# elfi-dev/elfi

Hardware: AMD Instinct MI355X
Metric: ABC distances/sec (higher is better)
Workload: dtype f64

## Files before the change

elfi_amd/csrc/gp_fit.hip:

```cpp
#include "gp.hpp"
#include "mfma_f64.hpp"
#include "sweep_sched.hpp"

#include <map>
#include <memory>
#include <mutex>

namespace elfihip {

struct GramArgs {
  const double* X;
  const double* x2;
  const double* y;
  double* A;
  int64_t lda, n, np;
  int dp;
  double var, neg_half_inv_ls2, bias, diag_add;
  int* info;
  int ninfo;
};

__global__ __launch_bounds__(256) void gram_kernel(GramArgs G) {
  extern __shared__ __align__(16) double sm[];
  const int pitch = G.dp + 1;
// ... 511 lines not shown
    } else {
      idx -= tA + m;
      const int r = idx / m;
      cblk = c0 + (idx - r * m);
      Ap = P.WT + ((int64_t)r * NB) * P.lda + (int64_t)P.ku0 * NB;
      C = P.WT + ((int64_t)r * NB) * P.lda + (int64_t)cblk * NB;
      beta0 = (r >= P.ku0);
    }
  }
  const double* Bp = P.A + ((int64_t)cblk * NB) * P.lda + (int64_t)P.ku0 * NB;
  GemmAcc acc;
  acc.zero();
  if (same)
    gemm_tile_nt<true>(acc, Ap, P.lda, Bp, P.lda, 0, P.kun * NB, lds);
  else
    gemm_tile_nt<false>(acc, Ap, P.lda, Bp, P.lda, 0, P.kun * NB, lds);
  if (beta0)
    acc_foreach(acc, [&](int row, int col, double v) { C[(int64_t)row * P.lda + col] = -v; });
  else
    acc_foreach(acc, [&](int row, int col, double v) { C[(int64_t)row * P.lda + col] -= v; });
}

__global__ __launch_bounds__(256) void trailing_update_col_kernel(PanelArgs P, int cblk) {
  extern __shared__ __align__(16) double lds[];
  cblk += blockIdx.y;
  const int rb = blockIdx.x >> 2, sub = blockIdx.x & 3;
  const int mrows = P.nb - cblk;
  if (rb >= mrows + 1 + P.ku0 + P.kun) return;
  const double* Ap;
  double* C;
  bool beta0 = false;
  if (rb < mrows) {
    const int ib = cblk + rb;
    Ap = P.A + ((int64_t)ib * NB) * P.lda + (int64_t)P.ku0 * NB;
    C = P.A + ((int64_t)ib * NB) * P.lda + (int64_t)cblk * NB;
  } else if (rb == mrows) {
    Ap = P.A + ((int64_t)P.nb * NB) * P.lda + (int64_t)P.ku0 * NB;
    C = P.A + ((int64_t)P.nb * NB) * P.lda + (int64_t)cblk * NB;
  } else {
    const int r = rb - mrows - 1;
    Ap = P.WT + ((int64_t)r * NB) * P.lda + (int64_t)P.ku0 * NB;
    C = P.WT + ((int64_t)r * NB) * P.lda + (int64_t)cblk * NB;
    beta0 = (r >= P.ku0);
  }
  Ap += (int64_t)sub * 32 * P.lda;
  C += (int64_t)sub * 32 * P.lda;
  const double* Bp = P.A + ((int64_t)cblk * NB) * P.lda + (int64_t)P.ku0 * NB;
  GemmAcc32 acc;
  acc.zero();
  gemm_tile32_nt(acc, Ap, P.lda, Bp, P.lda, 0, P.kun * NB, lds);
  if (beta0)
    acc32_foreach(acc, [&](int row, int col, double v) { C[(int64_t)row * P.lda + col] = -v; });
  else
    acc32_foreach(acc, [&](int row, int col, double v) { C[(int64_t)row * P.lda + col] -= v; });
}

template <int KUN, bool WT>
__device__ __forceinline__ void lookahead_tile_body(const PanelArgs& P, int cblk, int lb, double* lds) {
  const int t = threadIdx.x, l = t & 63, w = t >> 6;
  const int rb = lb >> 4, sub = (lb >> 2) & 3, cs = lb & 3;
  const int mrows = P.nb - cblk;
  if (rb >= mrows + 1 + P.ku0 + P.kun) return;
  const double* Ap;
  double* C;
  bool beta0 = false;
  if (rb < mrows) {
    const int ib = cblk + rb;
    Ap = P.A + ((int64_t)ib * NB) * P.lda + (int64_t)P.ku0 * NB;
    C = P.A + ((int64_t)ib * NB) * P.lda + (int64_t)cblk * NB;
  } else if (rb == mrows) {
    Ap = P.A + ((int64_t)P.nb * NB) * P.lda + (int64_t)P.ku0 * NB;
    C = P.A + ((int64_t)P.nb * NB) * P.lda + (int64_t)cblk * NB;
  } else {
    const int r = rb - mrows - 1;
    Ap = P.WT + ((int64_t)r * NB) * P.lda + (int64_t)P.ku0 * NB;
    C = P.WT + ((int64_t)r * NB) * P.lda + (int64_t)cblk * NB;
    beta0 = (r >= P.ku0);
  }
  Ap += (int64_t)sub * 32 * P.lda;
  C += (int64_t)sub * 32 * P.lda + cs * 32;
  const double* Bp = P.A + ((int64_t)cblk * NB + cs * 32) * P.lda + (int64_t)P.ku0 * NB;
  constexpr int KW = 32 * KUN;
  constexpr int NO = 4;
  const int kb = w * KW + 2 * (l >> 4);
  const double* pa = Ap + (int64_t)(l & 15) * P.lda + kb;
  const double* pb = Bp + (int64_t)(l & 15) * P.lda + kb;
  double2 a[2][2][NO], b[2][2][NO];
  auto load_piece = [&](int buf, int piece) {
#pragma unroll
    for (int o = 0; o < NO; ++o)
#pragma unroll
      for (int i = 0; i < 2; ++i) {
        a[buf][i][o] = *reinterpret_cast<const double2*>(pa + (int64_t)i * 16 * P.lda + 32 * piece + 8 * o);
        b[buf][i][o] = *reinterpret_cast<const double2*>(pb + (int64_t)i * 16 * P.lda + 32 * piece + 8 * o);
      }
  };
  load_piece(0, 0);
  if (KUN > 1) load_piece(1, 1);
  double cv[4];
#pragma unroll
  for (int u = 0; u < 4; ++u) {
    const int e = t + 256 * u;
    cv[u] = beta0 ? 0.0 : C[(int64_t)(e >> 5) * P.lda + (e & 31)];
  }
  v4d acc[2][2];
#pragma unroll
  for (int i = 0; i < 2; ++i)
#pragma unroll
    for (int j = 0; j < 2; ++j) acc[i][j] = (v4d){0.0, 0.0, 0.0, 0.0};
#pragma unroll
  for (int piece = 0; piece < KUN; ++piece) {
    const int buf = piece & 1;
#pragma unroll
    for (int o = 0; o < NO; ++o)
#pragma unroll
      for (int i = 0; i < 2; ++i)
#pragma unroll
        for (int j = 0; j < 2; ++j) {
          acc[i][j] = __builtin_amdgcn_mfma_f64_16x16x4f64(a[buf][i][o].x, b[buf][j][o].x, acc[i][j], 0, 0, 0);
          acc[i][j] = __builtin_amdgcn_mfma_f64_16x16x4f64(a[buf][i][o].y, b[buf][j][o].y, acc[i][j], 0, 0, 0);
        }
    if (piece + 2 < KUN) load_piece(buf, piece + 2);
  }
  constexpr int TP = 33;
  double* part = lds + w * 32 * TP;
#pragma unroll
  for (int i = 0; i < 2; ++i)
#pragma unroll
    for (int j = 0; j < 2; ++j)
#pragma unroll
      for (int r = 0; r < 4; ++r) part[(i * 16 + (l >> 4) + 4 * r) * TP + j * 16 + (l & 15)] = acc[i][j][r];
  __syncthreads();
#pragma unroll
  for (int u = 0; u < 4; ++u) {
    const int e = t + 256 * u;
    const int o = (e >> 5) * TP + (e & 31);
    const double s = ((lds[o] + lds[32 * TP + o]) + lds[2 * 32 * TP + o]) + lds[3 * 32 * TP + o];
    if (WT)
      store_wt_f64(C + (int64_t)(e >> 5) * P.lda + (e & 31), cv[u] - s);
    else
      C[(int64_t)(e >> 5) * P.lda + (e & 31)] = cv[u] - s;
  }
}

template <int KUN>
__global__ __launch_bounds__(256) void lookahead_tile_kernel(PanelArgs P, int cblk) {
  extern __shared__ __align__(16) double lds[];
  lookahead_tile_body<KUN, false>(P, cblk + blockIdx.y, (blockIdx.x & 7) * (gridDim.x >> 3) + (blockIdx.x >> 3), lds);
}
constexpr size_t LOOKAHEAD_TILE_LDS = 4 * 32 * 33 * sizeof(double);

constexpr int LOOK_TILES = 36;
constexpr int LOOK_PP = 130;
constexpr size_t PANEL_LOOK_LDS = (2 * 16 * LOOK_PP + 4 * 16 * 17) * sizeof(double);

template <int W>
__device__ __forceinline__ void look_strip_wave(const double* As, int64_t lda, const double* W11, int l, double* Ps,
                                                unsigned* cnt) {
  constexpr int T0 = W, T1 = 7 - W;
  constexpr int O0 = 2 * (T0 + 1), O1 = 2 * (T1 + 1);
  const int q2 = 2 * (l >> 4);
  const double* pa = As + (int64_t)(l & 15) * lda + q2;
  const double* pb0 = W11 + (int64_t)(16 * T0 + (l & 15)) * NB + q2;
  const double* pb1 = W11 + (int64_t)(16 * T1 + (l & 15)) * NB + q2;
  double2 a[O1], b0[O0], b1[O1];
#pragma unroll
  for (int o = 0; o < O1; ++o) a[o] = *reinterpret_cast<const double2*>(pa + 8 * o);
#pragma unroll
  for (int o = 0; o < O0; ++o) b0[o] = *reinterpret_cast<const double2*>(pb0 + 8 * o);
#pragma unroll
  for (int o = 0; o < O1; ++o) b1[o] = *reinterpret_cast<const double2*>(pb1 + 8 * o);
  __builtin_amdgcn_s_waitcnt(WAIT_VMCNT0);
  if (l == 0) __hip_atomic_fetch_add(cnt, 1u, __ATOMIC_RELAXED, __HIP_MEMORY_SCOPE_AGENT);
  v4d c0 = (v4d){0.0, 0.0, 0.0, 0.0}, c1 = c0;
#pragma unroll
  for (int o = 0; o < O1; ++o) {
    if (o < O0) {
      c0 = __builtin_amdgcn_mfma_f64_16x16x4f64(a[o].x, b0[o].x, c0, 0, 0, 0);
      c0 = __builtin_amdgcn_mfma_f64_16x16x4f64(a[o].y, b0[o].y, c0, 0, 0, 0);
    }
    c1 = __builtin_amdgcn_mfma_f64_16x16x4f64(a[o].x, b1[o].x, c1, 0, 0, 0);
    c1 = __builtin_amdgcn_mfma_f64_16x16x4f64(a[o].y, b1[o].y, c1, 0, 0, 0);
  }
  double* po = Ps + (l >> 4) * LOOK_PP + (l & 15);
#pragma unroll
  for (int r = 0; r < 4; ++r) {
    po[4 * r * LOOK_PP + 16 * T0] = c0[r];
    po[4 * r * LOOK_PP + 16 * T1] = c1[r];
  }
}

constexpr unsigned LOOK_ARRIVALS = 28u * 8u + 8u * 4u;

__global__ __launch_bounds__(512) void panel_look_kernel(PanelArgs P, unsigned* cnt, int* info) {
  extern __shared__ __align__(16) double lds[];
  const int t = threadIdx.x, l = t & 63, w = t >> 6, ww = w & 3, half = w >> 2;
  if (blockIdx.x >= LOOK_TILES) {
    const int piece = 2 * (blockIdx.x - LOOK_TILES) + half;
    const int npieces = 8 * P.nb;
    const int pc = piece < npieces ? piece : npieces - 1;
    double* Pb = panel_block(P, pc >> 3) + (int64_t)(pc & 7) * 16 * P.lda;
    unsigned* wait = (pc >> 3) == 0 ? cnt : nullptr;
    switch (ww) {
      case 0: trsm16_wave<0>(Pb, P.lda, P.W11, l, wait, info); break;
      case 1: trsm16_wave<1>(Pb, P.lda, P.W11, l, wait, info); break;
      case 2: trsm16_wave<2>(Pb, P.lda, P.W11, l, wait, info); break;
      default: trsm16_wave<3>(Pb, P.lda, P.W11, l, wait, info); break;
    }
    return;
  }
  int i = 0, b = blockIdx.x;
  while (b > i) {
    b -= i + 1;
    ++i;
  }
  const int j = b;
  const bool diag = i == j;
  const double* Ablk = P.A + ((int64_t)(P.k + 1) * NB) * P.lda + (int64_t)P.k * NB;
  double* C = P.A + ((int64_t)(P.k + 1) * NB + 16 * i) * P.lda + (int64_t)(P.k + 1) * NB + 16 * j;
  double* Pi = lds;
  double* Pj = diag ? lds : lds + 16 * LOOK_PP;
  double* part = lds + 2 * 16 * LOOK_PP;
  double cv = 0.0;
  if (t < 256) cv = C[(int64_t)(t >> 4) * P.lda + (t & 15)];
  if (half == 0 || !diag) {
    const double* As = Ablk + (int64_t)(16 * (half == 0 ? i : j)) * P.lda;
    double* Ps = half == 0 ? Pi : Pj;
    switch (ww) {
      case 0: look_strip_wave<0>(As, P.lda, P.W11, l, Ps, cnt); break;
      case 1: look_strip_wave<1>(As, P.lda, P.W11, l, Ps, cnt); break;
      case 2: look_strip_wave<2>(As, P.lda, P.W11, l, Ps, cnt); break;
      default: look_strip_wave<3>(As, P.lda, P.W11, l, Ps, cnt); break;
    }
  }
  __syncthreads();
  if (half == 0) {
    const int kb = 32 * w + 2 * (l >> 4);
    const double* pa = Pi + (l & 15) * LOOK_PP + kb;
    const double* pb = Pj + (l & 15) * LOOK_PP + kb;
    v4d acc = (v4d){0.0, 0.0, 0.0, 0.0};
#pragma unroll
    for (int o = 0; o < 4; ++o) {
      const double2 a = *reinterpret_cast<const double2*>(pa + 8 * o);
      const double2 bb = *reinterpret_cast<const double2*>(pb + 8 * o);
      acc = __builtin_amdgcn_mfma_f64_16x16x4f64(a.x, bb.x, acc, 0, 0, 0);
      acc = __builtin_amdgcn_mfma_f64_16x16x4f64(a.y, bb.y, acc, 0, 0, 0);
    }
#pragma unroll
    for (int r = 0; r < 4; ++r) part[w * 16 * 17 + ((l >> 4) + 4 * r) * 17 + (l & 15)] = acc[r];
  }
  __syncthreads();
  if (t < 256) {
    const int o = (t >> 4) * 17 + (t & 15);
    const double sum = ((part[o] + part[16 * 17 + o]) + part[2 * 16 * 17 + o]) + part[3 * 16 * 17 + o];
    C[(int64_t)(t >> 4) * P.lda + (t & 15)] = cv - sum;
  }
}

__device__ __noinline__ void potf2_tiles_call(double* Akk, int64_t lda, double* Wkk, int64_t ldw, double* W11, int* info,
                                              int kblock, double* sm) {
  potf2_tiles_body<1024>(Akk, lda, Wkk, ldw, W11, info, kblock, sm);
}
__device__ __noinline__ void potf2_tiles_call_wt(double* Akk, int64_t lda, double* Wkk, int64_t ldw, double* W11, int* info,
                                                 int kblock, double* sm) {
  potf2_tiles_body<1024, true>(Akk, lda, Wkk, ldw, W11, info, kblock, sm);
}

struct StepArgs {
  PanelArgs P;
  double* W11;
  int* info;
  const SweepUnit* units;
  const int32_t* wg_off;
  const SweepUnit* heads;
  unsigned* cnt;
  int nmini;
  int nwg;
};

struct StepUnit {
  const double* Ap;
  const double* Bp;
  double* C;
  double keep;
  int nkt;
  int kt0;
};

__device__ __forceinline__ StepUnit step_decode(const StepArgs& S, const int4 r) {
  const PanelArgs& P = S.P;
  const int row = r.x, c = r.y & 0xffff, kt0 = (r.y >> 16) & 0xffff;
  const int nkt = r.z & 0xffff, half = (r.z >> 16) & 0xff, keep = (r.z >> 24) & 0xff;
  const double* base = row <= P.nb ? P.A + ((int64_t)row * NB) * P.lda : P.WT + ((int64_t)(row - P.nb - 1) * NB) * P.lda;
  StepUnit U;
  U.Ap = base + (int64_t)kt0 * GK2 + (int64_t)half * 64 * P.lda;
  U.C = const_cast<double*>(base) + (int64_t)c * NB + (int64_t)half * 64 * P.lda;
  U.Bp = P.A + ((int64_t)c * NB) * P.lda + (int64_t)kt0 * GK2;
  U.keep = keep ? 1.0 : 0.0;
  U.nkt = nkt;
  U.kt0 = kt0;
  return U;
}

__device__ __forceinline__ StepUnit step_unit(const StepArgs& S, int i) {
  return step_decode(S, *reinterpret_cast<const int4*>(S.units + i));
}

#ifdef ELFIHIP_STEP_STAMP
__device__ long long g_step_stamp[1024 * 8];
__device__ int g_step_stamp_k = 16;
#define SSTAMP(slot) do { if (threadIdx.x == 0 && S.P.k == g_step_stamp_k) g_step_stamp[blockIdx.x * 8 + (slot)] = __builtin_readcyclecounter(); } while (0)
#else
#define SSTAMP(slot) do { } while (0)
#endif

constexpr int STEP_SPIN_LIMIT = 1 << 22;
constexpr int STEP_INFO_TIMEOUT = -1;

__device__ __forceinline__ void step_wait(const unsigned* c, unsigned target, int* info) {
  if (threadIdx.x < 64) {
    if (threadIdx.x == 0) {
      int spins = 0;
      while (__hip_atomic_load(c, __ATOMIC_RELAXED, __HIP_MEMORY_SCOPE_AGENT) < target) {
        if (++spins >= STEP_SPIN_LIMIT) {
          atomicCAS(info, 0, STEP_INFO_TIMEOUT);
          break;
        }
        __builtin_amdgcn_s_sleep(2);
      }
    }
    __builtin_amdgcn_fence(__ATOMIC_ACQUIRE, "agent");
  }
  __syncthreads();
}
__device__ __forceinline__ void step_arrive(unsigned* c, unsigned n, unsigned* c2 = nullptr) {
  asm volatile("s_waitcnt vmcnt(0)" ::: "memory");
  __syncthreads();
  if (threadIdx.x == 0) {
    __hip_atomic_fetch_add(c, n, __ATOMIC_RELAXED, __HIP_MEMORY_SCOPE_AGENT);
    if (c2) __hip_atomic_fetch_add(c2, n, __ATOMIC_RELAXED, __HIP_MEMORY_SCOPE_AGENT);
  }
}

__device__ __forceinline__ void step_solve_piece(const PanelArgs& P, int piece, double* sm) {
  double* Pb = panel_block(P, piece >> 3) + (int64_t)(piece & 7) * 16 * P.lda;
  const int l = threadIdx.x & 63, w = threadIdx.x >> 6;
  const int h = w >> 3, T = w & 7;
  const int O = 2 * (T + 1);
  const int q2 = 2 * (l >> 4);
  const double* pa = Pb + (int64_t)(l & 15) * P.lda + q2 + 64 * h;
  const double* pb = P.W11 + (int64_t)(16 * T + (l & 15)) * NB + q2 + 64 * h;
  double2 a[8], b[8];
#pragma unroll
  for (int j = 0; j < 8; ++j) {
    a[j] = (double2){0.0, 0.0};
    b[j] = (double2){0.0, 0.0};
    if (8 * h + j < O) {
      a[j] = *reinterpret_cast<const double2*>(pa + 8 * j);
      b[j] = *reinterpret_cast<const double2*>(pb + 8 * j);
    }
  }
  v4d c = (v4d){0.0, 0.0, 0.0, 0.0};
#pragma unroll
  for (int j = 0; j < 8; ++j)
    if (8 * h + j < O) {
      c = __builtin_amdgcn_mfma_f64_16x16x4f64(a[j].x, b[j].x, c, 0, 0, 0);
      c = __builtin_amdgcn_mfma_f64_16x16x4f64(a[j].y, b[j].y, c, 0, 0, 0);
    }
  double* part = sm + (T * 64 + l) * 4;
  if (h == 1) {
#pragma unroll
    for (int r = 0; r < 4; ++r) part[r] = c[r];
  }
  __syncthreads();
  if (h == 0) {
    double* po = Pb + (int64_t)(l >> 4) * P.lda + (l & 15) + 16 * T;
#pragma unroll
    for (int r = 0; r < 4; ++r) store_wt_f64(po + (int64_t)(4 * r) * P.lda, c[r] + part[r]);
  }
  __syncthreads();
}

__device__ __forceinline__ void step_tile_pieces(const PanelArgs& P, int pair, double* sm) {
  const int t = threadIdx.x & 255, l = t & 63, w = t >> 6;
  const int g = threadIdx.x >> 8;
  const int lb = 2 * pair + (g & 1);
  const int sub = (lb >> 2) & 3, cs = lb & 3;
  const int cblk = P.k + 1;
  constexpr int TP = 33;
  double* lds = sm + (g & 1) * 4 * 32 * TP;
  const bool on = g < 2;
  const double* Ap = P.A + ((int64_t)cblk * NB + sub * 32) * P.lda + (int64_t)P.k * NB;
  const double* Bp = P.A + ((int64_t)cblk * NB + cs * 32) * P.lda + (int64_t)P.k * NB;
  double* C = P.A + ((int64_t)cblk * NB + sub * 32) * P.lda + (int64_t)cblk * NB + cs * 32;
  double cv[4];
  if (on) {
    const int kb = w * 32 + 2 * (l >> 4);
    const double* pa = Ap + (int64_t)(l & 15) * P.lda + kb;
    const double* pb = Bp + (int64_t)(l & 15) * P.lda + kb;
    double2 a[2][4], b[2][4];
#pragma unroll
    for (int o = 0; o < 4; ++o)
#pragma unroll
      for (int i = 0; i < 2; ++i) {
        a[i][o] = *reinterpret_cast<const double2*>(pa + (int64_t)i * 16 * P.lda + 8 * o);
        b[i][o] = *reinterpret_cast<const double2*>(pb + (int64_t)i * 16 * P.lda + 8 * o);
      }
#pragma unroll
    for (int u = 0; u < 4; ++u) {
      const int e = t + 256 * u;
      cv[u] = C[(int64_t)(e >> 5) * P.lda + (e & 31)];
    }
    v4d acc[2][2];
#pragma unroll
    for (int i = 0; i < 2; ++i)
#pragma unroll
      for (int j = 0; j < 2; ++j) acc[i][j] = (v4d){0.0, 0.0, 0.0, 0.0};
#pragma unroll
    for (int o = 0; o < 4; ++o)
#pragma unroll
      for (int i = 0; i < 2; ++i)
#pragma unroll
        for (int j = 0; j < 2; ++j) {
          acc[i][j] = __builtin_amdgcn_mfma_f64_16x16x4f64(a[i][o].x, b[j][o].x, acc[i][j], 0, 0, 0);
          acc[i][j] = __builtin_amdgcn_mfma_f64_16x16x4f64(a[i][o].y, b[j][o].y, acc[i][j], 0, 0, 0);
        }
    double* part = lds + w * 32 * TP;
#pragma unroll
    for (int i = 0; i < 2; ++i)
#pragma unroll
      for (int j = 0; j < 2; ++j)
#pragma unroll
        for (int r = 0; r < 4; ++r) part[(i * 16 + (l >> 4) + 4 * r) * TP + j * 16 + (l & 15)] = acc[i][j][r];
  }
  __syncthreads();
  if (on) {
#pragma unroll
    for (int u = 0; u < 4; ++u) {
      const int e = t + 256 * u;
      const int o = (e >> 5) * TP + (e & 31);
      const double sres = ((lds[o] + lds[32 * TP + o]) + lds[2 * 32 * TP + o]) + lds[3 * 32 * TP + o];
      store_wt_f64(C + (int64_t)(e >> 5) * P.lda + (e & 31), cv[u] - sres);
    }
  }
}

template <bool CHAINED, bool WT>
__device__ __forceinline__ void step_units(const StepArgs& S, double* sm, int wgi) {
  const PanelArgs& P = S.P;
  constexpr bool chained = CHAINED;
  constexpr int RT = 1;
  constexpr int ROWS = 64 * RT;
  constexpr int BUF = (ROWS + 128) * GLP2;
  const int4 head = *reinterpret_cast<const int4*>(S.heads + wgi);
  int u = S.wg_off[wgi];
  if (head.w <= 0) return;
  const int uend = u + head.w;
  const int t = threadIdx.x, l = t & 63, w = t >> 6;
  const int wr = w >> 2, wc = w & 3;
  const int64_t lda = P.lda;
  const int64_t goff = (int64_t)(t >> 4) * lda + 2 * (t & 15);
  const int doff = (t >> 4) * GLP2 + 2 * (t & 15);
  const int faoff = (wr * 16 * RT + (l & 15)) * GLP2 + 2 * (l >> 4);
  const int fboff = (ROWS + wc * 32 + (l & 15)) * GLP2 + 2 * (l >> 4);
  const int64_t coff = (int64_t)(wr * 16 * RT + (l >> 4)) * lda + wc * 32 + (l & 15);

  StepUnit cur = step_decode(S, head);
  const int kt_new = chained ? 4 * P.k : (1 << 30);
  bool ready = !chained;
  auto need_panel = [&](const StepUnit& U, int kt) {
    if (chained && !ready && U.kt0 + kt >= kt_new) {
      SSTAMP(4);
      step_wait(S.cnt, (unsigned)S.nmini, S.info);
      SSTAMP(5);
      ready = true;
    }
  };
  double2 pa0, pa1, pb0, pb1;
  auto issue = [&](const double* A_, const double* B_) {
    pa0 = *reinterpret_cast<const double2*>(A_ + goff);
    if (RT == 2) pa1 = *reinterpret_cast<const double2*>(A_ + goff + 64 * lda);
    pb0 = *reinterpret_cast<const double2*>(B_ + goff);
    pb1 = *reinterpret_cast<const double2*>(B_ + goff + 64 * lda);
  };
  auto stage = [&](double* buf) {
    double* da = buf + doff;
    *reinterpret_cast<double2*>(da) = pa0;
    if (RT == 2) *reinterpret_cast<double2*>(da + 64 * GLP2) = pa1;
    *reinterpret_cast<double2*>(da + ROWS * GLP2) = pb0;
    *reinterpret_cast<double2*>(da + (ROWS + 64) * GLP2) = pb1;
  };
  pa1 = (double2){0.0, 0.0};
  need_panel(cur, 1);
  issue(cur.Ap, cur.Bp);
  v4d cv[RT][2];
#pragma unroll
  for (int i = 0; i < RT; ++i)
#pragma unroll
    for (int j = 0; j < 2; ++j)
#pragma unroll
      for (int r = 0; r < 4; ++r) cv[i][j][r] = cur.C[coff + (int64_t)(i * 16 + 4 * r) * lda + j * 16];
  int p = 0;
  stage(sm);
  issue(cur.Ap + GK2, cur.Bp + GK2);
  __syncthreads();
  for (;;) {
    const int un = u + 1;
    const bool more = un < uend;
    const StepUnit nxt = more ? step_unit(S, un) : cur;
    v4d acc[RT][2];
#pragma unroll
    for (int i = 0; i < RT; ++i)
#pragma unroll
      for (int j = 0; j < 2; ++j) acc[i][j] = (v4d){0.0, 0.0, 0.0, 0.0};
#pragma unroll 1
    for (int kt = 0; kt < cur.nkt; ++kt) {
      const double* buf = sm + p * BUF;
      if (kt + 1 < cur.nkt || more) {
        stage(sm + (p ^ 1) * BUF);
        const int k2 = kt + 2 - cur.nkt;
        if (k2 < 0) {
          need_panel(cur, kt + 2);
          issue(cur.Ap + (kt + 2) * GK2, cur.Bp + (kt + 2) * GK2);
        } else if (more) {
          need_panel(nxt, k2);
          issue(nxt.Ap + k2 * GK2, nxt.Bp + k2 * GK2);
        }
      }
      const double* fa = buf + faoff;
      const double* fb = buf + fboff;
#pragma unroll
      for (int h = 0; h < 4; ++h) {
        double2 a[RT], bb[2];
#pragma unroll
        for (int i = 0; i < RT; ++i) a[i] = *reinterpret_cast<const double2*>(fa + i * 16 * GLP2 + 8 * h);
#pragma unroll
        for (int j = 0; j < 2; ++j) bb[j] = *reinterpret_cast<const double2*>(fb + j * 16 * GLP2 + 8 * h);
#pragma unroll
        for (int i = 0; i < RT; ++i)
#pragma unroll
          for (int j = 0; j < 2; ++j) {
            acc[i][j] = __builtin_amdgcn_mfma_f64_16x16x4f64(a[i].x, bb[j].x, acc[i][j], 0, 0, 0);
            acc[i][j] = __builtin_amdgcn_mfma_f64_16x16x4f64(a[i].y, bb[j].y, acc[i][j], 0, 0, 0);
          }
      }
      __syncthreads();
      p ^= 1;
    }
    double* cp = cur.C + coff;
#pragma unroll
    for (int i = 0; i < RT; ++i)
#pragma unroll
      for (int j = 0; j < 2; ++j)
#pragma unroll
        for (int r = 0; r < 4; ++r)
          if (WT)
            store_wt_f64(cp + (int64_t)(i * 16 + 4 * r) * lda + j * 16, cur.keep * cv[i][j][r] - acc[i][j][r]);
          else
            cp[(int64_t)(i * 16 + 4 * r) * lda + j * 16] = cur.keep * cv[i][j][r] - acc[i][j][r];
    if (!more) {
      SSTAMP(6);
      break;
    }
    const double* cn = nxt.C + coff;
#pragma unroll
    for (int i = 0; i < RT; ++i)
#pragma unroll
      for (int j = 0; j < 2; ++j)
#pragma unroll
        for (int r = 0; r < 4; ++r) cv[i][j][r] = cn[(int64_t)(i * 16 + 4 * r) * lda + j * 16];
    cur = nxt;
    u = un;
  }
}

template <bool CHAINED>
__device__ __forceinline__ void step_body(const StepArgs& S) {
  extern __shared__ __align__(16) double sm[];
  const PanelArgs& P = S.P;
  constexpr bool chained = CHAINED;
  SSTAMP(0);
  if (blockIdx.x == 0) {
    const int kk = P.k + 1;
    double* Akk = P.A + ((int64_t)kk * NB) * P.lda + (int64_t)kk * NB;
    double* Wkk = P.WT + ((int64_t)kk * NB) * P.lda + (int64_t)kk * NB;
    if (chained) step_wait(S.cnt + 2, 8u, S.info);
    SSTAMP(1);
    if (S.W11) potf2_tiles_call(Akk, P.lda, Wkk, P.lda, S.W11, S.info, kk, sm);
    SSTAMP(2);
    return;
  }
  const int idx = blockIdx.x - 1;
  if (chained) {
    const int lead = S.nwg >= 16 ? 8 : 0;
    if (idx < 8) {
      step_solve_piece(P, idx, sm);
      step_arrive(S.cnt + 1, 1u, S.cnt);
      SSTAMP(1);
    }
    unsigned done = 0;
    if (idx >= lead)
      for (int e = 8 + (idx - lead); e < S.nmini; e += S.nwg - lead) {
        step_solve_piece(P, e, sm);
        ++done;
      }
    if (done) step_arrive(S.cnt, done);
    if (idx >= 8) SSTAMP(1);
    if (idx < 8) {
      step_wait(S.cnt + 1, 8u, S.info);
      SSTAMP(2);
      step_tile_pieces(P, idx, sm);
      step_arrive(S.cnt + 2, 1u);
      SSTAMP(3);
    }
  }
  step_units<CHAINED, false>(S, sm, idx);
}

__global__ __launch_bounds__(1024) void step_kernel(StepArgs S) { step_body<false>(S); }
__global__ __launch_bounds__(1024) void step_chain_kernel(StepArgs S) { step_body<true>(S); }

constexpr size_t STEP_LDS_BYTES = 2 * (64 + 128) * GLP2 * sizeof(double);
static_assert(STEP_LDS_BYTES >= POTF2T_LDS_DOUBLES * sizeof(double) && STEP_LDS_BYTES <= 160 * 1024, "LDS budget");

constexpr int OV_WORDS = 8;
constexpr int OV_POTF2 = 0, OV_PANEL = 1, OV_STRIP = 2, OV_TILE = 3, OV_UPD = 4;
constexpr int OV_AUX_XRANK = 0;
constexpr int OV_AUX_NEXT = 16;
constexpr int OV_AUX_DIAG_XCC = 17;
constexpr int OV_AUX_RESIDENT = 18;
constexpr int OV_AUX_WORDS = 32;
constexpr int OV_TILE_WGS = 16;
constexpr int OV_SPIN_LIMIT = 1 << 20;

__device__ __forceinline__ bool ov_poll(const unsigned* c, unsigned target, int* info, int who = 0) {
  int spins = 0;
  while (__hip_atomic_load(c, __ATOMIC_RELAXED, __HIP_MEMORY_SCOPE_AGENT) < target) {
    ++spins;
    if (spins >= OV_SPIN_LIMIT || ((spins & 31) == 0 && __hip_atomic_load(info + 1, __ATOMIC_RELAXED, __HIP_MEMORY_SCOPE_AGENT) != 0)) {
      if (atomicCAS(info + 1, 0, 1) == 0) {
        info[2] = who;
        info[3] = (int)((__hip_atomic_load(c, __ATOMIC_RELAXED, __HIP_MEMORY_SCOPE_AGENT) << 16) | (target & 0xffffu));
      }
      atomicCAS(info, 0, STEP_INFO_TIMEOUT);
      return false;
    }
    __builtin_amdgcn_s_sleep(8);
  }
  return true;
}
__device__ __forceinline__ bool ov_wait(const unsigned* c0, unsigned t0, const unsigned* c1, unsigned t1, int* info, int* s_ok,
                                        int who) {
  if (threadIdx.x < 64) {
    if (threadIdx.x == 0) {
      bool ok = ov_poll(c0, t0, info, who);
      if (ok && c1) ok = ov_poll(c1, t1, info, who + 1);
      *s_ok = ok ? 1 : 0;
    }
    __builtin_amdgcn_fence(__ATOMIC_ACQUIRE, "agent");
  }
  __syncthreads();
  return *s_ok != 0;
}
__device__ __forceinline__ void ov_arrive(unsigned* c, unsigned* c2 = nullptr) {
  asm volatile("s_waitcnt vmcnt(0)" ::: "memory");
  __syncthreads();
  if (threadIdx.x == 0) {
    __hip_atomic_fetch_add(c, 1u, __ATOMIC_RELAXED, __HIP_MEMORY_SCOPE_AGENT);
    if (c2) __hip_atomic_fetch_add(c2, 1u, __ATOMIC_RELAXED, __HIP_MEMORY_SCOPE_AGENT);
  }
}

struct OvArgs {
  PanelArgs P;
  double* W11;
  int* info;
  unsigned* flags;
  const SweepUnit* units;
  const int32_t* wg_off;
  const SweepUnit* heads;
  unsigned* aux;
  int nwg;
};

__device__ __forceinline__ unsigned ov_xcc_id() { return __builtin_amdgcn_s_getreg((3 << 11) | 20) & 15u; }

__global__ __launch_bounds__(1024) __attribute__((amdgpu_waves_per_eu(5))) void sweep_update_kernel(OvArgs O) {
  extern __shared__ __align__(16) double sm[];
  __shared__ int s_ok;
  __shared__ int s_wgi;
  if (threadIdx.x == 0) {
    __hip_atomic_fetch_add(O.aux + OV_AUX_XRANK + ov_xcc_id(), 1u, __ATOMIC_RELAXED, __HIP_MEMORY_SCOPE_AGENT);
    const int w = (int)__hip_atomic_fetch_add(O.aux + OV_AUX_NEXT, 1u, __ATOMIC_RELAXED, __HIP_MEMORY_SCOPE_AGENT);
    if (w < O.nwg) __hip_atomic_fetch_add(O.aux + OV_AUX_RESIDENT, 1u, __ATOMIC_RELAXED, __HIP_MEMORY_SCOPE_AGENT);
    s_wgi = w;
  }
  __syncthreads();
  const int wgi = s_wgi;
  if (wgi >= O.nwg) return;
  StepArgs S;
  S.P = O.P;
  S.P.kun = 1;
  S.W11 = nullptr;
  S.info = O.info;
  S.units = O.units;
  S.cnt = nullptr;
  S.nmini = 0;
  S.nwg = O.nwg;
  for (int k = 0; k + 1 < O.P.nb; ++k) {
    S.heads = O.heads + (size_t)k * O.nwg;
    const int4 head = *reinterpret_cast<const int4*>(S.heads + wgi);
    if (head.w <= 0) continue;
    unsigned* fl = O.flags + (size_t)OV_WORDS * k;
    if (!ov_wait(fl + OV_PANEL, 8u * (unsigned)O.P.nb, nullptr, 0u, O.info, &s_ok, 1000 + k)) return;
    S.P.k = k;
    S.P.ku0 = k;
    S.wg_off = O.wg_off + (size_t)k * (O.nwg + 1);
    step_units<false, true>(S, sm, wgi);
    ov_arrive(fl + OV_UPD);
  }
}

__global__ __launch_bounds__(1024) void sweep_diag_kernel(OvArgs O) {
  extern __shared__ __align__(16) double sm[];
  __shared__ int s_ok;
  const int wid = __builtin_amdgcn_readfirstlane(threadIdx.x >> 6);
  if (wid >= 11 || wid == 7 || wid == 8) return;
  if (threadIdx.x == 0) {
    __hip_atomic_store(O.aux + OV_AUX_DIAG_XCC, 1u + ov_xcc_id(), __ATOMIC_RELAXED, __HIP_MEMORY_SCOPE_AGENT);
    __hip_atomic_fetch_add(O.aux + OV_AUX_RESIDENT, 1u, __ATOMIC_RELAXED, __HIP_MEMORY_SCOPE_AGENT);
  }
  const PanelArgs& P = O.P;
  for (int k = 0; k + 1 < P.nb; ++k) {
    unsigned* fl = O.flags + (size_t)OV_WORDS * k;
    if (!ov_wait(fl + OV_TILE, (unsigned)OV_TILE_WGS, nullptr, 0u, O.info, &s_ok, 2000 + k)) return;
    const int kk = k + 1;
    double* Akk = P.A + ((int64_t)kk * NB) * P.lda + (int64_t)kk * NB;
    double* Wkk = P.WT + ((int64_t)kk * NB) * P.lda + (int64_t)kk * NB;
    potf2_tiles_call_wt(Akk, P.lda, Wkk, P.lda, O.W11 + (size_t)(kk & 1) * NB * NB, O.info, kk, sm);
    asm volatile("s_waitcnt vmcnt(0)" ::: "memory");
    __syncthreads();
    if (threadIdx.x == 0)
      __hip_atomic_store(fl + OV_WORDS + OV_POTF2, 1u, __ATOMIC_RELAXED, __HIP_MEMORY_SCOPE_AGENT);
  }
}

__global__ __launch_bounds__(256) __attribute__((amdgpu_waves_per_eu(4))) void chain_ov_kernel(PanelArgs P, unsigned* fl, unsigned upd_target, int ntile, int* info) {
  extern __shared__ __align__(16) double lds[];
  __shared__ int s_ok;
  __builtin_amdgcn_s_setprio(3);
  if ((int)blockIdx.x < ntile) {
    if (!ov_wait(fl + OV_STRIP, 8u, nullptr, 0u, info, &s_ok, 5000 + P.k)) return;
    lookahead_tile_body<1, true>(P, P.k + 1, blockIdx.x, lds);
    ov_arrive(fl + OV_TILE);
    return;
  }
  const int b = blockIdx.x - ntile;
  if (P.k > 0 && !ov_wait(fl + OV_POTF2, 1u, fl - OV_WORDS + OV_UPD, upd_target, info, &s_ok, 3000 + 2 * P.k)) return;
  double* Pb = panel_block(P, b >> 3) + (int64_t)(b & 7) * 16 * P.lda;
  const int l = threadIdx.x & 63;
  switch (threadIdx.x >> 6) {
    case 0: trsm16_wave<0, true>(Pb, P.lda, P.W11, l); break;
    case 1: trsm16_wave<1, true>(Pb, P.lda, P.W11, l); break;
    case 2: trsm16_wave<2, true>(Pb, P.lda, P.W11, l); break;
    default: trsm16_wave<3, true>(Pb, P.lda, P.W11, l); break;
  }
  ov_arrive(fl + OV_PANEL, (ntile && b < 8) ? fl + OV_STRIP : nullptr);
}

__global__ __launch_bounds__(64) void ov_gate_kernel(const unsigned* word, unsigned target, int* info, int who) {
  if (threadIdx.x == 0) ov_poll(word, target, info, who);
}

__global__ __launch_bounds__(256) void alpha_logdet_kernel(const double* WT, const double* A, const double* z, double* alpha,
                                                           double* red, const int* info, int64_t n, int64_t np, int64_t lda,
                                                           unsigned long long ticket) {
  if (blockIdx.x == 0) {
    __shared__ double s0[256], s1[256], s2[256], s3[256];
    double a = 0.0, b = 0.0, lo = 1e300, hi = 0.0;
    for (int64_t i = threadIdx.x; i < n; i += 256) {
      const double dg = A[i * lda + i];
      a += log(dg);
      b += z[i] * z[i];
      lo = dg < lo ? dg : lo;
      hi = dg > hi ? dg : hi;
    }
    s0[threadIdx.x] = a;
    s1[threadIdx.x] = b;
    s2[threadIdx.x] = lo;
    s3[threadIdx.x] = hi;
    __syncthreads();
    for (int off = 128; off > 0; off >>= 1) {
      if (threadIdx.x < off) {
        s0[threadIdx.x] += s0[threadIdx.x + off];
        s1[threadIdx.x] += s1[threadIdx.x + off];
        s2[threadIdx.x] = s2[threadIdx.x + off] < s2[threadIdx.x] ? s2[threadIdx.x + off] : s2[threadIdx.x];
        s3[threadIdx.x] = s3[threadIdx.x + off] > s3[threadIdx.x] ? s3[threadIdx.x + off] : s3[threadIdx.x];
      }
      __syncthreads();
    }
    if (threadIdx.x == 0) {
      red[0] = s0[0];
      red[1] = s1[0];
      red[2] = (double)*info;
      red[8] = s2[0];
      red[9] = s3[0];
      post_ticket(red + 15, ticket);
    }
    return;
  }
  const int lane = threadIdx.x & 63;
  const int64_t row = (int64_t)(blockIdx.x - 1) * 4 + (threadIdx.x >> 6);
  double s = 0.0;
  if (row < n) {
    const double* w = WT + row * lda;
    double p[8] = {0.0, 0.0, 0.0, 0.0, 0.0, 0.0, 0.0, 0.0};
    int64_t k = (row & ~(int64_t)63) + lane;
    for (; k + 7 * 64 < n; k += 512) {
      double wv[8], zv[8];
#pragma unroll
      for (int u = 0; u < 8; ++u) {
        wv[u] = w[k + 64 * u];
        zv[u] = z[k + 64 * u];
      }
#pragma unroll
      for (int u = 0; u < 8; ++u) p[u] += (k + 64 * u >= row) ? wv[u] * zv[u] : 0.0;
    }
    double tail = 0.0;
    for (; k < n; k += 64)
      if (k >= row) tail += w[k] * z[k];
    s = (((p[0] + p[1]) + (p[2] + p[3])) + ((p[4] + p[5]) + (p[6] + p[7]))) + tail;
#pragma unroll
    for (int off = 32; off > 0; off >>= 1) s += __shfl_xor(s, off, 64);
  }
  if (lane == 0 && row < np) alpha[row] = s;
}

template <class K>
static int enable_lds(elfihip_ctx* ctx, K k, size_t bytes) {
  ELFIHIP_CHECK_HIP(ctx, hipFuncSetAttribute(reinterpret_cast<const void*>(k),
                                             hipFuncAttributeMaxDynamicSharedMemorySize, (int)bytes));
  return ELFIHIP_OK;
}

static std::mutex g_sched_mutex;
static std::map<std::pair<int, int>, std::shared_ptr<const SweepSchedule>> g_sched_cache;

static std::shared_ptr<const SweepSchedule> sweep_schedule_for(int nb, int nwg, bool far_first) {
  std::lock_guard<std::mutex> lock(g_sched_mutex);
  auto key = std::make_pair(nb, far_first ? -nwg : nwg);
  auto it = g_sched_cache.find(key);
  if (it != g_sched_cache.end()) return it->second;
  auto S = std::make_shared<SweepSchedule>();
  sweep_build(nb, nwg, S.get(), far_first);
  g_sched_cache[key] = S;
  return S;
}

static int sweep_plan(elfihip_gp* gp, int nb, int nwg, bool far_first, hipStream_t st) {
  if (gp->sched_nb == nb && gp->sched_nwg == nwg && gp->sched_far_first == far_first) return ELFIHIP_OK;
  elfihip_ctx* ctx = gp->ctx;
  std::shared_ptr<const SweepSchedule> S = sweep_schedule_for(nb, nwg, far_first);
  std::vector<SweepUnit> heads;
  for (const SweepStep& x : S->steps)
    for (int w = 0; w < nwg; ++w) {
      const int lo = S->wg_off[x.off0 + w], hi = S->wg_off[x.off0 + w + 1];
      SweepUnit h = {};
      if (hi > lo) h = S->units[lo];
      heads.push_back(h);
    }
  const size_t ub = S->units.size() * sizeof(SweepUnit), ob = S->wg_off.size() * sizeof(int32_t);
  const size_t hb = heads.size() * sizeof(SweepUnit);
  ELFIHIP_CHECK_HIP(ctx, hipStreamSynchronize(st));
// ... 596 lines not shown
```

Baseline: 22.30 billion.

## Defer tile epilogue stores into next unit's k-loop and load schedule via constant address space

In the non-write-through step path, a finished unit's C tile result is no longer stored right away. It is kept in registers and written during the first k-iteration of the next unit, after that iteration's prefetch has been issued. The next unit's C values are loaded at that same point, so the store and load latency overlaps with MFMA work instead of stalling between units. Schedule records and offsets are also read through address-space-4 (constant) pointers, which should allow scalar loads. The cost is extra live registers for the deferred result, and correctness now depends on the next unit not needing the deferred tile before it is stored.

```diff
diff --git a/elfi_amd/csrc/gp_fit.hip b/elfi_amd/csrc/gp_fit.hip
--- a/elfi_amd/csrc/gp_fit.hip
+++ b/elfi_amd/csrc/gp_fit.hip
@@ -837,8 +837,16 @@
   return U;
 }
 
+typedef int kv4i_t __attribute__((ext_vector_type(4)));
+typedef __attribute__((address_space(4))) const kv4i_t kint4;
+typedef __attribute__((address_space(4))) const int32_t kint32;
+__device__ __forceinline__ int4 sched_record(const SweepUnit* p) {
+  const kv4i_t r = *(kint4*)p;
+  return make_int4(r.x, r.y, r.z, r.w);
+}
+
 __device__ __forceinline__ StepUnit step_unit(const StepArgs& S, int i) {
-  return step_decode(S, *reinterpret_cast<const int4*>(S.units + i));
+  return step_decode(S, sched_record(S.units + i));
 }
 
 #ifdef ELFIHIP_STEP_STAMP
@@ -987,8 +995,8 @@
   constexpr int RT = 1;
   constexpr int ROWS = 64 * RT;
   constexpr int BUF = (ROWS + 128) * GLP2;
-  const int4 head = *reinterpret_cast<const int4*>(S.heads + wgi);
-  int u = S.wg_off[wgi];
+  const int4 head = sched_record(S.heads + wgi);
+  int u = *(kint32*)(S.wg_off + wgi);
   if (head.w <= 0) return;
   const int uend = u + head.w;
   const int t = threadIdx.x, l = t & 63, w = t >> 6;
@@ -1039,6 +1047,29 @@
   stage(sm);
   issue(cur.Ap + GK2, cur.Bp + GK2);
   __syncthreads();
+  constexpr bool DEFER = !WT;
+  auto put = [&](double* dst, const v4d (&v)[RT][2]) {
+#pragma unroll
+    for (int i = 0; i < RT; ++i)
+#pragma unroll
+      for (int j = 0; j < 2; ++j)
+#pragma unroll
+        for (int r = 0; r < 4; ++r)
+          if (WT)
+            store_wt_f64(dst + (int64_t)(i * 16 + 4 * r) * lda + j * 16, v[i][j][r]);
+          else
+            dst[(int64_t)(i * 16 + 4 * r) * lda + j * 16] = v[i][j][r];
+  };
+  auto load_c = [&](const double* src) {
+#pragma unroll
+    for (int i = 0; i < RT; ++i)
+#pragma unroll
+      for (int j = 0; j < 2; ++j)
+#pragma unroll
+        for (int r = 0; r < 4; ++r) cv[i][j][r] = src[(int64_t)(i * 16 + 4 * r) * lda + j * 16];
+  };
+  v4d res[RT][2];
+  double* rp = nullptr;
   for (;;) {
     const int un = u + 1;
     const bool more = un < uend;
@@ -1062,6 +1093,11 @@
           issue(nxt.Ap + k2 * GK2, nxt.Bp + k2 * GK2);
         }
       }
+      if (DEFER && rp) {
+        put(rp, res);
+        rp = nullptr;
+        load_c(cur.C + coff);
+      }
       const double* fa = buf + faoff;
       const double* fb = buf + fboff;
 #pragma unroll
@@ -1082,28 +1118,22 @@
       __syncthreads();
       p ^= 1;
     }
-    double* cp = cur.C + coff;
 #pragma unroll
     for (int i = 0; i < RT; ++i)
 #pragma unroll
       for (int j = 0; j < 2; ++j)
 #pragma unroll
-        for (int r = 0; r < 4; ++r)
-          if (WT)
-            store_wt_f64(cp + (int64_t)(i * 16 + 4 * r) * lda + j * 16, cur.keep * cv[i][j][r] - acc[i][j][r]);
-          else
-            cp[(int64_t)(i * 16 + 4 * r) * lda + j * 16] = cur.keep * cv[i][j][r] - acc[i][j][r];
-    if (!more) {
-      SSTAMP(6);
-      break;
-    }
-    const double* cn = nxt.C + coff;
-#pragma unroll
-    for (int i = 0; i < RT; ++i)
-#pragma unroll
-      for (int j = 0; j < 2; ++j)
-#pragma unroll
-        for (int r = 0; r < 4; ++r) cv[i][j][r] = cn[(int64_t)(i * 16 + 4 * r) * lda + j * 16];
+        for (int r = 0; r < 4; ++r) res[i][j][r] = cur.keep * cv[i][j][r] - acc[i][j][r];
+    if (DEFER && more) {
+      rp = cur.C + coff;
+    } else {
+      put(cur.C + coff, res);
+      if (!more) {
+        SSTAMP(6);
+        break;
+      }
+      load_c(nxt.C + coff);
+    }
     cur = nxt;
     u = un;
   }
```

Result: no change. 22.35 billion (median of 6 runs) (+0.2%).
